# tsurumeso/vocal-remover

Measured on NVIDIA H100. Metric: seconds-of-audio/sec separated (n_fft=2048, hop=1024), higher is better.
Workload: dtype bf16x3 (split-bf16 operands hi+lo, 3 wgmma passes, fp32 accumulate); fft/lstm fp32

## Files before the change

vocal-remover_b200/build.py:

```python
import os
import subprocess
import sys
from concurrent.futures import ThreadPoolExecutor

HERE = os.path.dirname(os.path.abspath(__file__))
CSRC = os.path.join(HERE, 'csrc')
OBJ = os.path.join(HERE, 'build')
LIB = os.path.join(HERE, 'libvr_b200.so')
SOURCES = ['api.cu', 'engine.cu', 'conv_simt.cu', 'conv_tc.cu', 'conv_tc_rows.cu', 'elementwise.cu', 'lstm.cu', 'fft.cu', 'resample.cu']
NVCC = os.environ.get('NVCC', '/usr/local/cuda/bin/nvcc')
FLAGS = ['-gencode', 'arch=compute_90a,code=sm_90a', '-O3', '-lineinfo', '-std=c++17',
         '-Xcompiler', '-fPIC', '-Xcompiler', '-fvisibility=hidden', '--expt-relaxed-constexpr']


def _newest_header():
    hs = [os.path.join(CSRC, f) for f in os.listdir(CSRC) if f.endswith(('.h', '.cuh'))]
    hs.append(os.path.join(HERE, '..', 'include', 'vr_b200.h'))
    return max(os.path.getmtime(h) for h in hs)


def build(verbose=False, force=False):
    global OBJ, LIB
    extra = os.environ.get('VR_BUILD_FLAGS', '').split()
    if os.environ.get('VR_BUILD_TAG'):
        OBJ = os.path.join(HERE, 'build_' + os.environ['VR_BUILD_TAG'])
        LIB = os.path.join(HERE, 'libvr_b200_%s.so' % os.environ['VR_BUILD_TAG'])
    os.makedirs(OBJ, exist_ok=True)
    hdr = _newest_header()
    jobs = []
    for src in SOURCES:
        s = os.path.join(CSRC, src)
        o = os.path.join(OBJ, src.replace('.cu', '.o'))
        if force or not os.path.exists(o) or os.path.getmtime(o) < max(os.path.getmtime(s), hdr):
            jobs.append((s, o))

    def cc(job):
        s, o = job
        cmd = [NVCC] + FLAGS + extra + ['-c', s, '-o', o]
        if verbose:
            cmd += ['-Xptxas', '-v']
        r = subprocess.run(cmd, capture_output=True, text=True)
        if r.returncode != 0:
            raise RuntimeError('nvcc failed for %s:\n%s\n%s' % (s, r.stdout, r.stderr))
        return r.stderr

    with ThreadPoolExecutor(max_workers=min(8, max(1, len(jobs)))) as ex:
        logs = list(ex.map(cc, jobs))
    if verbose:
        for lg in logs:
            print(lg)
    objs = [os.path.join(OBJ, s.replace('.cu', '.o')) for s in SOURCES]
    if jobs or not os.path.exists(LIB):
        cmd = [NVCC, '-shared', '-o', LIB] + objs + ['-gencode', 'arch=compute_90a,code=sm_90a']
        r = subprocess.run(cmd, capture_output=True, text=True)
        if r.returncode != 0:
            raise RuntimeError('link failed:\n%s\n%s' % (r.stdout, r.stderr))
    return LIB


if __name__ == '__main__':
    print(build(verbose='-v' in sys.argv, force='-f' in sys.argv))
```

vocal-remover_b200/csrc/conv_tc.cu:

```cuda
#include <cuda.h>
#include <stdio.h>

#include <map>
#include <tuple>

#include "engine.h"
#include "tc_common.cuh"
#include "tc_plan.h"

namespace vr {

static constexpr int kMaxStages = 8;
static constexpr int kConsumerWarps = 8;
static constexpr int kThreads = 32 * kConsumerWarps + 32;

struct TcParams {
  int N, Ho, Wo, Wt, Ht, Nt, tiles_w, tiles_h, m_tiles, n_tiles;
  int stride, pad_h, pad_w, dil_h, dil_w, KW;
  int cchunks, total_sub, CinPadTC, Cout, act, stages;
  bf16* out_hi;
  bf16* out_lo;
  int64_t osn, osh;
  int osw;
  const float* bias;
// ... 117 lines not shown
        if (++stage == p.stages) {
          stage = 0;
          phase ^= 1u;
        }
      }
      wg_wait<0>();
      __syncwarp();
      if (lane == 0) mbar_arrive(empty0 + (uint32_t)prev * 8u);

      const int nt = tile % p.n_tiles;
      const int mt = tile / p.n_tiles;
      const int w0 = (mt % p.tiles_w) * p.Wt;
      const int h0 = ((mt / p.tiles_w) % p.tiles_h) * p.Ht;
      const int n0 = (mt / (p.tiles_w * p.tiles_h)) * p.Nt;
      const int c_lane = nt * BN + 2 * (lane & 3);
#pragma unroll
      for (int hr = 0; hr < 2; ++hr) {
        const int row = 64 * wg + 16 * (warp & 3) + (lane >> 2) + 8 * hr;
        const int dw = row % p.Wt;
        const int dh = (row / p.Wt) % p.Ht;
        const int n = n0 + row / (p.Wt * p.Ht);
        if (n >= p.N) continue;
        const int64_t obase = (int64_t)n * p.osn + (int64_t)(h0 + dh) * p.osh + (int64_t)(w0 + dw) * p.osw;
#pragma unroll
        for (int j = 0; j < BN / 8; ++j)
          epilogue_pair(acc[4 * j + 2 * hr], acc[4 * j + 2 * hr + 1], bias_s, c_lane + 8 * j, p.Cout, slope,
                        p.out_hi + obase, p.out_lo + obase);
      }
    }
  }
}

#define VR_TC_FOR_BN(X, KB) X(KB, 16) X(KB, 32) X(KB, 48) X(KB, 64) X(KB, 80) X(KB, 96) X(KB, 112) X(KB, 128)
#define VR_TC_FOR_ALL(X) VR_TC_FOR_BN(X, 64) VR_TC_FOR_BN(X, 32) VR_TC_FOR_BN(X, 16)

int g_tc_debug[8] = {0, 0, 0, 0, 0, 1, 1, 0};

static constexpr int kMaxDevices = 64;
const TcDevice& tc_device() {
  static TcDevice table[kMaxDevices];
  static TcDevice none;
  int dev = -1;
  if (cudaGetDevice(&dev) != cudaSuccess || dev < 0 || dev >= kMaxDevices) return none;
  TcDevice& d = table[dev];
  if (!d.ok) {
    if (cudaDeviceGetAttribute(&d.max_smem, cudaDevAttrMaxSharedMemoryPerBlockOptin, dev) != cudaSuccess ||
        cudaDeviceGetAttribute(&d.num_sms, cudaDevAttrMultiProcessorCount, dev) != cudaSuccess)
      return none;
#define VR_TC_SET_SMEM(KB, BN) \
  cudaFuncSetAttribute(conv_tc_kernel<KB, BN>, cudaFuncAttributeMaxDynamicSharedMemorySize, d.max_smem - 2048);
    VR_TC_FOR_ALL(VR_TC_SET_SMEM)
#undef VR_TC_SET_SMEM
    tc_rows_set_attributes(d.max_smem);
    d.ok = true;
  }
  return d;
}

EncodeTiledFn tc_encode_fn() {
  static EncodeTiledFn fn = nullptr;
  if (!fn) {
    void* p = nullptr;
    cudaDriverEntryPointQueryResult q;
    if (cudaGetDriverEntryPoint("cuTensorMapEncodeTiled", &p, cudaEnableDefault, &q) == cudaSuccess &&
        q == cudaDriverEntryPointSuccess)
      fn = (EncodeTiledFn)p;
  }
  return fn;
}

static CUtensorMapSwizzle swizzle_for(int KB) {
  return KB == 64 ? CU_TENSOR_MAP_SWIZZLE_128B : KB == 32 ? CU_TENSOR_MAP_SWIZZLE_64B : CU_TENSOR_MAP_SWIZZLE_32B;
}

uint16_t tc_f2bf(float f) {
  uint32_t u;
  memcpy(&u, &f, 4);
  if ((u & 0x7fffffffu) > 0x7f800000u) return (uint16_t)((u >> 16) | 0x40);
  uint32_t r = 0x7fffu + ((u >> 16) & 1u);
  return (uint16_t)((u + r) >> 16);
}
float tc_bf2f(uint16_t h) {
  uint32_t u = (uint32_t)h << 16;
  float f;
  memcpy(&f, &u, 4);
  return f;
}

struct TileGeom {
  int Wt, Ht, Nt;
  bool ok;
};
static TileGeom tile_geom(int Ho, int Wo) {
  TileGeom g{0, 0, 0, false};
  if (Wo <= 0 || Ho <= 0) return g;
  if (Wo >= 128) {
    if (Wo % 128) return g;
    g.Wt = 128; g.Ht = 1; g.Nt = 1;
  } else {
    if (128 % Wo) return g;
    g.Wt = Wo;
    g.Ht = 128 / Wo < Ho ? 128 / Wo : Ho;
    if (Ho % g.Ht) return g;
    if ((128 / Wo) % g.Ht) return g;
    g.Nt = 128 / (g.Wt * g.Ht);
  }
// ... 27 lines not shown
  auto tc = std::make_shared<TcConv>();
  tc->taps = L.k * L.k;
  tc->CinPadTC = round_up(L.CinPad, 16);
  tc->KB = tc->CinPadTC % 64 == 0 ? 64 : tc->CinPadTC % 32 == 0 ? 32 : 16;
  tc->cchunks = tc->CinPadTC / tc->KB;
  tc->SUBS = 64 / tc->KB;
  tc->Ktot = tc->taps * tc->CinPadTC;
  tc->CoutPadN = round_up(L.Cout, 16);
  tc->n_tiles = ceil_div(tc->CoutPadN, 128);
  tc->BN = round_up(ceil_div(tc->CoutPadN, tc->n_tiles), 16);
  const int rows = tc->n_tiles * tc->BN;
  std::vector<uint16_t> planes((size_t)2 * rows * tc->Ktot, 0);
  for (int co = 0; co < L.Cout; ++co)
    for (int t = 0; t < tc->taps; ++t)
      for (int ci = 0; ci < L.CinPad; ++ci) {
        const float w = L.w_host[((size_t)t * L.CinPad + ci) * L.CoutPad + co];
        const uint16_t hi = tc_f2bf(w);
        const uint16_t lo = tc_f2bf(w - tc_bf2f(hi));
        const size_t k = (size_t)t * tc->CinPadTC + ci;
        planes[(size_t)co * tc->Ktot + k] = hi;
        planes[((size_t)rows + co) * tc->Ktot + k] = lo;
      }
  std::vector<float> bias((size_t)rows, 0.f);
  for (int co = 0; co < L.Cout; ++co) bias[(size_t)co] = L.bias_host[(size_t)co];
  void* dw = nullptr;
  void* db = nullptr;
  if (cudaMalloc(&dw, planes.size() * 2) != cudaSuccess || cudaMalloc(&db, bias.size() * 4) != cudaSuccess) {
    err = "cudaMalloc failed while packing tensor-core weights for " + L.name;
    return false;
  }
  allocs.push_back(dw);
  allocs.push_back(db);
  cudaMemcpy(dw, planes.data(), planes.size() * 2, cudaMemcpyHostToDevice);
  cudaMemcpy(db, bias.data(), bias.size() * 4, cudaMemcpyHostToDevice);
  tc->w_planes = (bf16*)dw;
  tc->bias = (float*)db;
  EncodeTiledFn enc = tc_encode_fn();
  if (!enc) {
    err = "cuTensorMapEncodeTiled is not available from the driver";
    return false;
  }
  cuuint64_t dims[3] = {(cuuint64_t)tc->Ktot, (cuuint64_t)rows, 2};
  cuuint64_t strides[2] = {(cuuint64_t)tc->Ktot * 2, (cuuint64_t)rows * tc->Ktot * 2};
  cuuint32_t box[3] = {(cuuint32_t)tc->KB, (cuuint32_t)tc->BN, 2};
  cuuint32_t es[3] = {1, 1, 1};
  CUresult r = enc(&tc->map_b, CU_TENSOR_MAP_DATA_TYPE_BFLOAT16, 3, dw, dims, strides, box, es,
                   CU_TENSOR_MAP_INTERLEAVE_NONE, swizzle_for(tc->KB), CU_TENSOR_MAP_L2_PROMOTION_L2_256B,
                   CU_TENSOR_MAP_FLOAT_OOB_FILL_NONE);
  if (r != CUDA_SUCCESS) {
    err = "cuTensorMapEncodeTiled(weights) failed for " + L.name + " code " + std::to_string((int)r);
    return false;
  }
  if (!tc_rows_prepare(L, *tc, err, allocs)) return false;
  L.tc = tc;
  return true;
}

cudaError_t tc_launch(ConvLayer& L, const ActView& in, const ActView& out, cudaStream_t s, std::string& err,
                      const ActView* up_src, const ActView* extra) {
  TcConv& tc = *L.tc;
  if (tc_rows_supported(L, tc, in, out)) return tc_rows_launch(L, tc, in, out, s, err, up_src, extra);
  if (up_src || extra) {
    err = "tc_launch: fused upsample is only implemented in the row-streaming kernel";
    return cudaErrorInvalidValue;
  }
  const TileGeom g = tile_geom(out.H, out.W);
  auto key = std::make_tuple((const void*)in.hi, (const void*)in.lo, in.N, in.H, in.W, in.C);
  auto it = tc.map_a.find(key);
  if (it == tc.map_a.end()) {
    CUtensorMap m;
    cuuint64_t dims[5] = {(cuuint64_t)in.C, (cuuint64_t)in.W, (cuuint64_t)in.H, (cuuint64_t)in.N, 2};
    const int64_t plane = (const char*)in.lo - (const char*)in.hi;
    if (plane <= 0 || plane % 16) {
      err = "tc_launch: hi/lo planes must be 16-byte aligned with lo after hi";
      return cudaErrorInvalidValue;
    }
    cuuint64_t strides[4] = {(cuuint64_t)in.sw * 2, (cuuint64_t)in.sh * 2, (cuuint64_t)in.sn * 2, (cuuint64_t)plane};
    cuuint32_t box[5] = {(cuuint32_t)tc.KB, (cuuint32_t)(g.Wt * L.stride), (cuuint32_t)(g.Ht * L.stride),
                         (cuuint32_t)g.Nt, 2};
    cuuint32_t es[5] = {1, (cuuint32_t)L.stride, (cuuint32_t)L.stride, 1, 1};
    CUresult r = tc_encode_fn()(&m, CU_TENSOR_MAP_DATA_TYPE_BFLOAT16, 5, (void*)in.hi, dims, strides, box, es,
                             CU_TENSOR_MAP_INTERLEAVE_NONE, swizzle_for(tc.KB), CU_TENSOR_MAP_L2_PROMOTION_L2_256B,
                             CU_TENSOR_MAP_FLOAT_OOB_FILL_NONE);
    if (r != CUDA_SUCCESS) {
      err = "cuTensorMapEncodeTiled(activations) failed for " + L.name + " code " + std::to_string((int)r);
      return cudaErrorInvalidValue;
    }
    it = tc.map_a.emplace(key, m).first;
  }
  TcParams p;
  p.N = out.N; p.Ho = out.H; p.Wo = out.W;
  p.Wt = g.Wt; p.Ht = g.Ht; p.Nt = g.Nt;
  p.tiles_w = out.W / g.Wt; p.tiles_h = out.H / g.Ht;
  p.m_tiles = p.tiles_w * p.tiles_h * ceil_div(out.N, g.Nt);
  p.n_tiles = tc.n_tiles;
  p.stride = L.stride; p.dil_h = L.dil_h; p.dil_w = L.dil_w;
  p.pad_h = L.dil_h * (L.k / 2); p.pad_w = L.dil_w * (L.k / 2);
  p.KW = L.k;
  p.cchunks = tc.cchunks; p.total_sub = tc.taps * tc.cchunks;
  p.CinPadTC = tc.CinPadTC; p.Cout = L.Cout; p.act = L.act;
  const int stage_bytes = tc.SUBS * (2 * 128 * tc.KB * 2 + 2 * tc.BN * tc.KB * 2);
  const TcDevice& dv = tc_device();
  if (!dv.ok) {
    err = "tc_launch: cannot query the current device";
    return cudaErrorInvalidValue;
  }
  const int dyn = dv.max_smem - 2048;
  p.stages = (dyn - 1024) / stage_bytes;
  if (p.stages > kMaxStages) p.stages = kMaxStages;
  if (p.stages < 2) {
    err = "tc_launch: shared memory too small for two pipeline stages";
    return cudaErrorInvalidValue;
  }
  p.out_hi = out.hi; p.out_lo = out.lo;
  p.osn = out.sn; p.osh = out.sh; p.osw = out.sw;
  p.bias = tc.bias;
  const int total_tiles = p.m_tiles * p.n_tiles;
  const int grid = total_tiles < dv.num_sms ? total_tiles : dv.num_sms;
// ... 13 lines not shown
```

vocal-remover_b200/csrc/conv_tc_rows.cu:

```cuda
#include <stdio.h>

#include "engine.h"
#include "tc_common.cuh"
#include "tc_plan.h"

namespace vr {

static constexpr int kInterpWarps = 10;
static constexpr int kConsumerWarps = 8;
static constexpr int kTmaWarp = kConsumerWarps;
static constexpr int kInterpWarp0 = kConsumerWarps + 1;
static constexpr int kMaxR = 8;
__host__ __device__ constexpr int rows_per_tile(int BN) { return BN == 64 ? 2 : BN == 32 ? 4 : 8; }
static constexpr int kUpProducerWarps = 12;
static constexpr int kUpConsumerRegs = 128;
static constexpr int kUpProducerRegs = 72;
static constexpr int kUpLaunchRegs = 96;
static_assert(kConsumerWarps * kUpConsumerRegs + kUpProducerWarps * kUpProducerRegs <=
                  (kConsumerWarps + kUpProducerWarps) * kUpLaunchRegs,
              "setmaxnreg.inc would wait forever for registers the block does not own");
__host__ __device__ constexpr int rows_threads(bool up) { return 32 * (kConsumerWarps + (up ? kUpProducerWarps : 1)); }
static constexpr int kRowPx = 130;
static constexpr int kBoxPx = 136;
static constexpr int kMaxASlots = 8;
static constexpr int kSrcPx = 68;
static constexpr uint32_t kKB = 32;
static constexpr uint32_t kRowB = kKB * 2;
static constexpr uint32_t kAPlane = kBoxPx * kRowB;
static constexpr uint32_t kASlot = 2 * kAPlane;

static constexpr int kTraceEvents = 2048;
__device__ unsigned long long g_rows_trace[3 * kTraceEvents * 3];

template <int BN>
struct RowsGeom {
  static constexpr uint32_t kBPlane = 3 * BN * kRowB;
  static constexpr uint32_t kBKw = 2 * kBPlane;
  static constexpr uint32_t kBBuf = 3 * kBKw;
};

struct RowsParams {
  int N, H, W, tiles_w, tiles_h, n_tiles, total_tiles;
  int chunks, CinPadR, Cout, act;
  int n_aslots;
  bf16* out_hi;
  bf16* out_lo;
  int64_t osn, osh;
  int osw;
  const float* bias;
  int up_chunks, xH, xW;
  const bf16* x_hi;
  const bf16* x_lo;
  int64_t xsn, xsh;
  int xsw;
  int trace;
  unsigned long long kmask;
  int a_c_off;
  int l_chunk;
  int n_uslots;
  float up_sh, up_sw;
  const float* dot_w;
  float* dot_out;
};

__device__ __forceinline__ uint32_t chunk_groups(unsigned long long kmask, int cc) {
  const int sh = cc * 4;
  return sh + 4 <= 64 ? (uint32_t)(kmask >> sh) & 0xFu : 0xFu;
}

struct RowsConsumer {
  int as_t, as_u, bs, as, pend_b;
  uint32_t aph_t, aph_u, bph, aph;
  int ring_lo, ring_hi;
};

template <int BN, int R, int r>
__device__ __forceinline__ void consume_rows(RowsConsumer& st, float* acc, uint32_t (&fr)[2][16], uint32_t lrow,
                                             uint32_t bsrc, uint32_t dhi, uint32_t ksm, uint32_t afull0,
                                             uint32_t aempty0, uint32_t bempty0, int lane) {
  constexpr int o_lo = r - 2 < 0 ? 0 : r - 2;
  constexpr int o_hi = r > R - 1 ? R - 1 : r;
  mbar_wait(afull0 + (uint32_t)st.as * 8u, st.aph);
  const uint32_t row = lrow + (uint32_t)st.as * kASlot;
#pragma unroll
  for (int kw = 0; kw < 3; ++kw) {
    uint32_t* f = fr[(3 * r + kw) & 1];
    const uint32_t q = (row >> 6) + (uint32_t)kw;
#pragma unroll
    for (int ks = 0; ks < 2; ++ks) {
      if (!((ksm >> ks) & 1u)) continue;
      const uint32_t a = (q << 6) + ((((uint32_t)(2 * ks) + ((uint32_t)lane >> 4)) ^ ((q >> 1) & 3u)) << 4);
      ldsm_x4(f + 8 * ks, a);
      ldsm_x4(f + 8 * ks + 4, a + kAPlane);
    }
    wg_fence();
#pragma unroll
    for (int ks = 0; ks < 2; ++ks) {
      if (!((ksm >> ks) & 1u)) continue;
      const uint32_t bo = (uint32_t)(kw * RowsGeom<BN>::kBKw + ks * 32) >> 4;
#pragma unroll
      for (int o = o_lo; o <= o_hi; ++o) {
        const uint32_t b_row = bsrc + (((uint32_t)((2 - (r - o)) * BN) * kRowB) >> 4) + bo;
        wgmma_split3_rs<BN>(acc + o * (BN / 2), f + 8 * ks, f + 8 * ks + 4, b_row,
                            b_row + (RowsGeom<BN>::kBPlane >> 4), dhi);
      }
    }
    wg_commit();
    if (kw == 2) {
      __syncwarp();
      if (lane == 0) mbar_arrive(aempty0 + (uint32_t)st.as * 8u);
    }
    wg_wait<1>();
    if (st.pend_b >= 0) {
      __syncwarp();
      if (lane == 0) mbar_arrive(bempty0 + (uint32_t)st.pend_b * 8u);
      st.pend_b = -1;
    }
  }
  if (++st.as == st.ring_hi) {
    st.as = st.ring_lo;
    st.aph ^= 1u;
// ... 543 lines not shown
```

vocal-remover_b200/csrc/tc_common.cuh:

```cuda
#pragma once
#include <cuda.h>
#include <stdint.h>
#include <stdio.h>

#include "common.cuh"

namespace vr {

__device__ __forceinline__ uint32_t smem_u32(const void* p) { return (uint32_t)__cvta_generic_to_shared(p); }

__device__ __forceinline__ bool elect_one_sync() {
  uint32_t pred;
  asm volatile(
      "{\n\t"
      ".reg .pred P1;\n\t"
      "elect.sync _|P1, 0xffffffff;\n\t"
      "selp.u32 %0, 1, 0, P1;\n\t"
      "}"
      : "=r"(pred));
  return pred != 0;
}

__device__ __forceinline__ void mbar_init(uint32_t bar, uint32_t count) {
  asm volatile("mbarrier.init.shared::cta.b64 [%0], %1;" ::"r"(bar), "r"(count));
// ... 130 lines not shown
  }
};
template <>
struct Wgmma<112> {
  static __device__ __forceinline__ void mma(float* d, uint64_t a, uint64_t b) {
    asm volatile(
        "wgmma.mma_async.sync.aligned.m64n112k16.f32.bf16.bf16 {%0, %1, %2, %3, %4, %5, %6, %7, %8, %9, %10, %11, %12, %13, %14, %15, %16, %17, %18, %19, %20, %21, %22, %23, %24, %25, %26, %27, %28, %29, %30, %31, %32, %33, %34, %35, %36, %37, %38, %39, %40, %41, %42, %43, %44, %45, %46, %47, %48, %49, %50, %51, %52, %53, %54, %55}, %56, %57, 1, 1, 1, 0, 0;"
        : "+f"(d[0]), "+f"(d[1]), "+f"(d[2]), "+f"(d[3]), "+f"(d[4]), "+f"(d[5]), "+f"(d[6]), "+f"(d[7]), "+f"(d[8]), "+f"(d[9]), "+f"(d[10]), "+f"(d[11]), "+f"(d[12]), "+f"(d[13]), "+f"(d[14]), "+f"(d[15]), "+f"(d[16]), "+f"(d[17]), "+f"(d[18]), "+f"(d[19]), "+f"(d[20]), "+f"(d[21]), "+f"(d[22]), "+f"(d[23]), "+f"(d[24]), "+f"(d[25]), "+f"(d[26]), "+f"(d[27]), "+f"(d[28]), "+f"(d[29]), "+f"(d[30]), "+f"(d[31]), "+f"(d[32]), "+f"(d[33]), "+f"(d[34]), "+f"(d[35]), "+f"(d[36]), "+f"(d[37]), "+f"(d[38]), "+f"(d[39]), "+f"(d[40]), "+f"(d[41]), "+f"(d[42]), "+f"(d[43]), "+f"(d[44]), "+f"(d[45]), "+f"(d[46]), "+f"(d[47]), "+f"(d[48]), "+f"(d[49]), "+f"(d[50]), "+f"(d[51]), "+f"(d[52]), "+f"(d[53]), "+f"(d[54]), "+f"(d[55])
        : "l"(a), "l"(b)
        : "memory");
  }
};
template <>
struct Wgmma<128> {
  static __device__ __forceinline__ void mma(float* d, uint64_t a, uint64_t b) {
    asm volatile(
        "wgmma.mma_async.sync.aligned.m64n128k16.f32.bf16.bf16 {%0, %1, %2, %3, %4, %5, %6, %7, %8, %9, %10, %11, %12, %13, %14, %15, %16, %17, %18, %19, %20, %21, %22, %23, %24, %25, %26, %27, %28, %29, %30, %31, %32, %33, %34, %35, %36, %37, %38, %39, %40, %41, %42, %43, %44, %45, %46, %47, %48, %49, %50, %51, %52, %53, %54, %55, %56, %57, %58, %59, %60, %61, %62, %63}, %64, %65, 1, 1, 1, 0, 0;"
        : "+f"(d[0]), "+f"(d[1]), "+f"(d[2]), "+f"(d[3]), "+f"(d[4]), "+f"(d[5]), "+f"(d[6]), "+f"(d[7]), "+f"(d[8]), "+f"(d[9]), "+f"(d[10]), "+f"(d[11]), "+f"(d[12]), "+f"(d[13]), "+f"(d[14]), "+f"(d[15]), "+f"(d[16]), "+f"(d[17]), "+f"(d[18]), "+f"(d[19]), "+f"(d[20]), "+f"(d[21]), "+f"(d[22]), "+f"(d[23]), "+f"(d[24]), "+f"(d[25]), "+f"(d[26]), "+f"(d[27]), "+f"(d[28]), "+f"(d[29]), "+f"(d[30]), "+f"(d[31]), "+f"(d[32]), "+f"(d[33]), "+f"(d[34]), "+f"(d[35]), "+f"(d[36]), "+f"(d[37]), "+f"(d[38]), "+f"(d[39]), "+f"(d[40]), "+f"(d[41]), "+f"(d[42]), "+f"(d[43]), "+f"(d[44]), "+f"(d[45]), "+f"(d[46]), "+f"(d[47]), "+f"(d[48]), "+f"(d[49]), "+f"(d[50]), "+f"(d[51]), "+f"(d[52]), "+f"(d[53]), "+f"(d[54]), "+f"(d[55]), "+f"(d[56]), "+f"(d[57]), "+f"(d[58]), "+f"(d[59]), "+f"(d[60]), "+f"(d[61]), "+f"(d[62]), "+f"(d[63])
        : "l"(a), "l"(b)
        : "memory");
  }
};
template <int N>
__device__ __forceinline__ void wgmma_split3(float* d, uint32_t a_hi, uint32_t a_lo, uint32_t b_hi, uint32_t b_lo,
                                             uint32_t dhi) {
  Wgmma<N>::mma(d, desc64(a_hi, dhi), desc64(b_hi, dhi));
  Wgmma<N>::mma(d, desc64(a_lo, dhi), desc64(b_hi, dhi));
  Wgmma<N>::mma(d, desc64(a_hi, dhi), desc64(b_lo, dhi));
}

template <int N>
struct WgmmaRS;
template <>
struct WgmmaRS<16> {
  static __device__ __forceinline__ void mma(float* d, const uint32_t* a, uint64_t b) {
    asm volatile(
        "wgmma.mma_async.sync.aligned.m64n16k16.f32.bf16.bf16 {%0, %1, %2, %3, %4, %5, %6, %7}, {%8, %9, %10, %11}, %12, 1, 1, 1, 0;"
        : "+f"(d[0]), "+f"(d[1]), "+f"(d[2]), "+f"(d[3]), "+f"(d[4]), "+f"(d[5]), "+f"(d[6]), "+f"(d[7])
        : "r"(a[0]), "r"(a[1]), "r"(a[2]), "r"(a[3]), "l"(b)
        : "memory");
  }
};
template <>
struct WgmmaRS<32> {
  static __device__ __forceinline__ void mma(float* d, const uint32_t* a, uint64_t b) {
    asm volatile(
        "wgmma.mma_async.sync.aligned.m64n32k16.f32.bf16.bf16 {%0, %1, %2, %3, %4, %5, %6, %7, %8, %9, %10, %11, %12, %13, %14, %15}, {%16, %17, %18, %19}, %20, 1, 1, 1, 0;"
        : "+f"(d[0]), "+f"(d[1]), "+f"(d[2]), "+f"(d[3]), "+f"(d[4]), "+f"(d[5]), "+f"(d[6]), "+f"(d[7]), "+f"(d[8]), "+f"(d[9]), "+f"(d[10]), "+f"(d[11]), "+f"(d[12]), "+f"(d[13]), "+f"(d[14]), "+f"(d[15])
        : "r"(a[0]), "r"(a[1]), "r"(a[2]), "r"(a[3]), "l"(b)
        : "memory");
  }
};
template <>
struct WgmmaRS<64> {
  static __device__ __forceinline__ void mma(float* d, const uint32_t* a, uint64_t b) {
    asm volatile(
        "wgmma.mma_async.sync.aligned.m64n64k16.f32.bf16.bf16 {%0, %1, %2, %3, %4, %5, %6, %7, %8, %9, %10, %11, %12, %13, %14, %15, %16, %17, %18, %19, %20, %21, %22, %23, %24, %25, %26, %27, %28, %29, %30, %31}, {%32, %33, %34, %35}, %36, 1, 1, 1, 0;"
        : "+f"(d[0]), "+f"(d[1]), "+f"(d[2]), "+f"(d[3]), "+f"(d[4]), "+f"(d[5]), "+f"(d[6]), "+f"(d[7]), "+f"(d[8]), "+f"(d[9]), "+f"(d[10]), "+f"(d[11]), "+f"(d[12]), "+f"(d[13]), "+f"(d[14]), "+f"(d[15]), "+f"(d[16]), "+f"(d[17]), "+f"(d[18]), "+f"(d[19]), "+f"(d[20]), "+f"(d[21]), "+f"(d[22]), "+f"(d[23]), "+f"(d[24]), "+f"(d[25]), "+f"(d[26]), "+f"(d[27]), "+f"(d[28]), "+f"(d[29]), "+f"(d[30]), "+f"(d[31])
        : "r"(a[0]), "r"(a[1]), "r"(a[2]), "r"(a[3]), "l"(b)
        : "memory");
  }
};
template <int N>
__device__ __forceinline__ void wgmma_split3_rs(float* d, const uint32_t* a_hi, const uint32_t* a_lo, uint32_t b_hi,
                                                uint32_t b_lo, uint32_t dhi) {
  WgmmaRS<N>::mma(d, a_hi, desc64(b_hi, dhi));
  WgmmaRS<N>::mma(d, a_lo, desc64(b_hi, dhi));
  WgmmaRS<N>::mma(d, a_hi, desc64(b_lo, dhi));
}

__device__ __forceinline__ void ldsm_x4(uint32_t* r, uint32_t addr) {
  asm volatile("ldmatrix.sync.aligned.m8n8.x4.shared.b16 {%0, %1, %2, %3}, [%4];"
               : "=r"(r[0]), "=r"(r[1]), "=r"(r[2]), "=r"(r[3])
               : "r"(addr)
               : "memory");
}

template <int N>
__device__ __forceinline__ void setmaxnreg_inc() {
  asm volatile("setmaxnreg.inc.sync.aligned.u32 %0;" ::"n"(N));
}
template <int N>
__device__ __forceinline__ void setmaxnreg_dec() {
  asm volatile("setmaxnreg.dec.sync.aligned.u32 %0;" ::"n"(N));
}

__device__ __forceinline__ void epilogue_pair(float v0, float v1, const float* bias_s, int c, int Cout, float slope,
                                              bf16* out_hi, bf16* out_lo) {
  if (c >= Cout) return;
  const float t0 = v0 + bias_s[c], t1 = v1 + bias_s[c + 1];
  const float y0 = fmaxf(t0, 0.f) + slope * fminf(t0, 0.f);
  const float y1 = fmaxf(t1, 0.f) + slope * fminf(t1, 0.f);
  bf16* h = out_hi + c;
  bf16* l = out_lo + c;
  if (c + 1 < Cout && ((reinterpret_cast<uintptr_t>(h) | reinterpret_cast<uintptr_t>(l)) & 3) == 0) {
    const uint32_t uh = f2_to_bf2(y0, y1);
    const float2 hf = bf2_to_f2(uh);
    *reinterpret_cast<uint32_t*>(h) = uh;
    *reinterpret_cast<uint32_t*>(l) = f2_to_bf2(y0 - hf.x, y1 - hf.y);
  } else {
    split_bf16(y0, h[0], l[0]);
    if (c + 1 < Cout) split_bf16(y1, h[1], l[1]);
  }
}

__device__ __forceinline__ void tma_load_4d(uint32_t dst, const CUtensorMap* map, int c0, int c1, int c2, int c3,
                                            uint32_t bar) {
  asm volatile(
      "cp.async.bulk.tensor.4d.shared::cluster.global.tile.mbarrier::complete_tx::bytes [%0], [%1, {%2, %3, %4, %5}], "
      "[%6];" ::"r"(dst),
      "l"(map), "r"(c0), "r"(c1), "r"(c2), "r"(c3), "r"(bar)
      : "memory");
}

}
```

vocal-remover_b200/csrc/tc_plan.h:

```cpp
#pragma once
#include <cuda.h>

#include <map>
#include <tuple>

#include "engine.h"

namespace vr {

typedef std::tuple<const void*, const void*, int, int, int, int> ViewKey;

struct TcRowsPlan {
  bool ok = false;
  int KB = 32, CinPadR = 0, chunks = 0, BN = 0, n_tiles = 0;
  unsigned long long kmask = ~0ull;
  bf16* w_planes = nullptr;
  float* bias = nullptr;
  CUtensorMap map_b;
  std::map<ViewKey, CUtensorMap> map_a;
  std::map<ViewKey, CUtensorMap> map_l;
};

struct TcConv {
  int CinPadTC = 0, KB = 0, cchunks = 0, SUBS = 0, taps = 0, Ktot = 0, CoutPadN = 0, BN = 0, n_tiles = 0;
  bf16* w_planes = nullptr;
  float* bias = nullptr;
  CUtensorMap map_b;
  std::map<ViewKey, CUtensorMap> map_a;
  TcRowsPlan rows;
};

typedef CUresult (*EncodeTiledFn)(CUtensorMap*, CUtensorMapDataType, cuuint32_t, void*, const cuuint64_t*,
                                  const cuuint64_t*, const cuuint32_t*, const cuuint32_t*, CUtensorMapInterleave,
                                  CUtensorMapSwizzle, CUtensorMapL2promotion, CUtensorMapFloatOOBfill);
EncodeTiledFn tc_encode_fn();
uint16_t tc_f2bf(float f);
float tc_bf2f(uint16_t h);

bool tc_rows_prepare(ConvLayer& L, TcConv& tc, std::string& err, std::vector<void*>& allocs);
bool tc_rows_supported(const ConvLayer& L, const TcConv& tc, const ActView& in, const ActView& out);
cudaError_t tc_rows_launch(ConvLayer& L, TcConv& tc, const ActView& in, const ActView& out, cudaStream_t s,
                           std::string& err, const ActView* up_src = nullptr, const ActView* extra = nullptr);
void tc_rows_set_attributes(int max_smem);
int tc_rows_read_trace(unsigned long long* out, long long capacity);

struct TcDevice {
  bool ok = false;
  int num_sms = 0, max_smem = 0;
};
const TcDevice& tc_device();

extern int g_tc_debug[8];

}
```

Before: 2613.

## Add halo-tile 3x3 conv kernel reusing one activation tile across all nine taps

Adds a new warp-specialized tensor-core kernel for 3x3 stride-1 convs on narrow widths (16/32/64). It loads one halo tile per channel chunk via TMA, builds all nine tap fragments from shared memory with ldmatrix, and streams the weights through a deep stage ring. This replaces per-tap re-fetching of activations in the generic implicit-GEMM path. It also chooses between one and two M-blocks per tile based on wave count. The new path is untested on other shapes, carries a large register budget, and adds more template instantiations.

```diff
diff --git a/vocal-remover_b200/build.py b/vocal-remover_b200/build.py
--- a/vocal-remover_b200/build.py
+++ b/vocal-remover_b200/build.py
@@ -7,7 +7,7 @@
 CSRC = os.path.join(HERE, 'csrc')
 OBJ = os.path.join(HERE, 'build')
 LIB = os.path.join(HERE, 'libvr_b200.so')
-SOURCES = ['api.cu', 'engine.cu', 'conv_simt.cu', 'conv_tc.cu', 'conv_tc_rows.cu', 'elementwise.cu', 'lstm.cu', 'fft.cu', 'resample.cu']
+SOURCES = ['api.cu', 'engine.cu', 'conv_simt.cu', 'conv_tc.cu', 'conv_tc_rows.cu', 'conv_tc_halo.cu', 'elementwise.cu', 'lstm.cu', 'fft.cu', 'resample.cu']
 NVCC = os.environ.get('NVCC', '/usr/local/cuda/bin/nvcc')
 FLAGS = ['-gencode', 'arch=compute_90a,code=sm_90a', '-O3', '-lineinfo', '-std=c++17',
          '-Xcompiler', '-fPIC', '-Xcompiler', '-fvisibility=hidden', '--expt-relaxed-constexpr']
diff --git a/vocal-remover_b200/csrc/conv_tc.cu b/vocal-remover_b200/csrc/conv_tc.cu
--- a/vocal-remover_b200/csrc/conv_tc.cu
+++ b/vocal-remover_b200/csrc/conv_tc.cu
@@ -193,6 +193,7 @@
     VR_TC_FOR_ALL(VR_TC_SET_SMEM)
 #undef VR_TC_SET_SMEM
     tc_rows_set_attributes(d.max_smem);
+    tc_halo_set_attributes(d.max_smem);
     d.ok = true;
   }
   return d;
@@ -326,6 +327,7 @@
     return false;
   }
   if (!tc_rows_prepare(L, *tc, err, allocs)) return false;
+  if (!tc_halo_prepare(L, *tc, err, allocs)) return false;
   L.tc = tc;
   return true;
 }
@@ -338,6 +340,7 @@
     err = "tc_launch: fused upsample is only implemented in the row-streaming kernel";
     return cudaErrorInvalidValue;
   }
+  if (tc_halo_supported(L, tc, in, out)) return tc_halo_launch(L, tc, in, out, s, err);
   const TileGeom g = tile_geom(out.H, out.W);
   auto key = std::make_tuple((const void*)in.hi, (const void*)in.lo, in.N, in.H, in.W, in.C);
   auto it = tc.map_a.find(key);
diff --git a/vocal-remover_b200/csrc/conv_tc_halo.cu b/vocal-remover_b200/csrc/conv_tc_halo.cu
--- /dev/null
+++ b/vocal-remover_b200/csrc/conv_tc_halo.cu
@@ -0,0 +1,372 @@
+#include <stdio.h>
+
+#include "engine.h"
+#include "tc_common.cuh"
+#include "tc_plan.h"
+
+namespace vr {
+
+static constexpr int kConsumerWarps = 8;
+static constexpr int kProducerWarps = 4;
+static constexpr int kThreads = 32 * (kConsumerWarps + kProducerWarps);
+static constexpr int kLaunchRegs = 168;
+static constexpr int kConsumerRegs = 232;
+static constexpr int kProducerRegs = 40;
+static_assert(kConsumerWarps * kConsumerRegs + kProducerWarps * kProducerRegs <=
+                  (kConsumerWarps + kProducerWarps) * kLaunchRegs,
+              "setmaxnreg.inc would wait forever for registers the block does not own");
+static constexpr int kMaxHSlots = 4;
+static constexpr int kMaxWStages = 18;
+static constexpr uint32_t kKB = 32;
+static constexpr uint32_t kRowB = kKB * 2;
+
+template <int BN>
+struct HaloGeom {
+  static constexpr uint32_t kBPlane = BN * kRowB;
+  static constexpr uint32_t kWStage = 2 * kBPlane;
+};
+
+struct HaloParams {
+  int N, H, W, lw, Ht, Wb, tiles_h, n_tiles, total_tiles;
+  int chunks, CinPadH, Cout, act;
+  int n_hslots, n_wstages;
+  uint32_t hplane, hslot;
+  unsigned long long kmask;
+  bf16* out_hi;
+  bf16* out_lo;
+  int64_t osn, osh;
+  int osw;
+  const float* bias;
+};
+
+struct HaloConsumer {
+  int hs, ws, pend_w;
+  uint32_t hph, wph;
+};
+
+template <int BN, int MB>
+__device__ __forceinline__ void consume_halo(HaloConsumer& st, const HaloParams& p, float* acc,
+                                             uint32_t (&fr)[2][MB * 8], const uint32_t* q0, uint32_t h_base,
+                                             uint32_t w_base, uint32_t dhi, uint32_t hfull0,
+                                             uint32_t hempty0, uint32_t wfull0, uint32_t wempty0, int lane) {
+  typedef HaloGeom<BN> G;
+  mbar_wait(hfull0 + (uint32_t)st.hs * 8u, st.hph);
+  const uint32_t slot = h_base + (uint32_t)st.hs * p.hslot;
+#pragma unroll
+  for (int t = 0; t < 9; ++t) {
+    const int kh = t / 3, kw = t % 3;
+#pragma unroll
+    for (int ks = 0; ks < 2; ++ks) {
+      uint32_t* f = fr[ks];
+#pragma unroll
+      for (int b = 0; b < MB; ++b) {
+        const uint32_t q = q0[b] + (uint32_t)(kh * p.Wb + kw);
+        const uint32_t a = slot + (q << 6) + ((((uint32_t)(2 * ks) + ((uint32_t)lane >> 4)) ^ ((q >> 1) & 3u)) << 4);
+        ldsm_x4(f + 8 * b, a);
+        ldsm_x4(f + 8 * b + 4, a + p.hplane);
+      }
+      if (ks == 0) mbar_wait(wfull0 + (uint32_t)st.ws * 8u, st.wph);
+      const uint32_t b_hi = desc_lo(w_base + (uint32_t)st.ws * G::kWStage) + (uint32_t)(ks * 32 >> 4);
+      wg_fence();
+#pragma unroll
+      for (int b = 0; b < MB; ++b)
+        wgmma_split3_rs<BN>(acc + b * (BN / 2), f + 8 * b, f + 8 * b + 4, b_hi, b_hi + (G::kBPlane >> 4), dhi);
+      wg_commit();
+      if (t == 8 && ks == 1) {
+        __syncwarp();
+        if (lane == 0) mbar_arrive(hempty0 + (uint32_t)st.hs * 8u);
+      }
+      wg_wait<1>();
+      if (st.pend_w >= 0) {
+        __syncwarp();
+        if (lane == 0) mbar_arrive(wempty0 + (uint32_t)st.pend_w * 8u);
+        st.pend_w = -1;
+      }
+    }
+    st.pend_w = st.ws;
+    if (++st.ws == p.n_wstages) {
+      st.ws = 0;
+      st.wph ^= 1u;
+    }
+  }
+  if (++st.hs == p.n_hslots) {
+    st.hs = 0;
+    st.hph ^= 1u;
+  }
+}
+
+template <int BN, int MB>
+__global__ void __launch_bounds__(kThreads, 1)
+    conv_tc_halo_kernel(const __grid_constant__ CUtensorMap tmA, const __grid_constant__ CUtensorMap tmB,
+                        const HaloParams p) {
+  typedef HaloGeom<BN> G;
+  extern __shared__ uint8_t smem_raw[];
+  __shared__ __align__(8) uint64_t bar_hfull[kMaxHSlots];
+  __shared__ __align__(8) uint64_t bar_hempty[kMaxHSlots];
+  __shared__ __align__(8) uint64_t bar_wfull[kMaxWStages];
+  __shared__ __align__(8) uint64_t bar_wempty[kMaxWStages];
+  __shared__ float bias_s[256];
+
+  const int warp = __shfl_sync(0xffffffffu, (int)threadIdx.x >> 5, 0);
+  const int lane = threadIdx.x & 31;
+  const uint32_t smem_base = (smem_u32(smem_raw) + 1023u) & ~1023u;
+  const uint32_t h_base = smem_base;
+  const uint32_t w_base = smem_base + (uint32_t)p.n_hslots * p.hslot;
+
+  if (warp == kConsumerWarps && lane == 0) {
+    asm volatile("prefetch.tensormap [%0];" ::"l"(&tmA) : "memory");
+    asm volatile("prefetch.tensormap [%0];" ::"l"(&tmB) : "memory");
+    for (int s = 0; s < p.n_hslots; ++s) {
+      mbar_init(smem_u32(&bar_hfull[s]), 1);
+      mbar_init(smem_u32(&bar_hempty[s]), kConsumerWarps);
+    }
+    for (int s = 0; s < p.n_wstages; ++s) {
+      mbar_init(smem_u32(&bar_wfull[s]), 1);
+      mbar_init(smem_u32(&bar_wempty[s]), kConsumerWarps);
+    }
+    asm volatile("fence.mbarrier_init.release.cluster;" ::: "memory");
+  }
+  for (int i = threadIdx.x; i < p.n_tiles * BN; i += blockDim.x) bias_s[i] = __ldg(p.bias + i);
+  __syncthreads();
+  const uint32_t hfull0 = smem_u32(&bar_hfull[0]), hempty0 = smem_u32(&bar_hempty[0]);
+  const uint32_t wfull0 = smem_u32(&bar_wfull[0]), wempty0 = smem_u32(&bar_wempty[0]);
+
+  if (warp >= kConsumerWarps) {
+    setmaxnreg_dec<kProducerRegs>();
+    if (warp == kConsumerWarps && elect_one_sync()) {
+      int hs = 0, ws = 0;
+      uint32_t hph = 0, wph = 0;
+      for (int tile = blockIdx.x; tile < p.total_tiles; tile += gridDim.x) {
+        const int nt = tile % p.n_tiles;
+        const int mt = tile / p.n_tiles;
+        const int h0 = (mt % p.tiles_h) * p.Ht;
+        const int n = mt / p.tiles_h;
+        for (int cc = 0; cc < p.chunks; ++cc) {
+          if (!chunk_groups(p.kmask, cc)) continue;
+          mbar_wait(hempty0 + (uint32_t)hs * 8u, hph ^ 1u);
+          const uint32_t hfull = hfull0 + (uint32_t)hs * 8u;
+          mbar_expect_tx(hfull, p.hslot);
+          tma_load_5d(h_base + (uint32_t)hs * p.hslot, &tmA, cc * (int)kKB, -1, h0 - 1, n, 0, hfull);
+          if (++hs == p.n_hslots) {
+            hs = 0;
+            hph ^= 1u;
+          }
+          for (int t = 0; t < 9; ++t) {
+            mbar_wait(wempty0 + (uint32_t)ws * 8u, wph ^ 1u);
+            const uint32_t wfull = wfull0 + (uint32_t)ws * 8u;
+            mbar_expect_tx(wfull, G::kWStage);
+            tma_load_3d(w_base + (uint32_t)ws * G::kWStage, &tmB, t * p.CinPadH + cc * (int)kKB, nt * BN, 0, wfull);
+            if (++ws == p.n_wstages) {
+              ws = 0;
+              wph ^= 1u;
+            }
+          }
+        }
+      }
+    }
+    __syncwarp();
+  } else {
+    setmaxnreg_inc<kConsumerRegs>();
+    const int wg = warp >> 2;
+    const float slope = p.act == ACT_RELU ? 0.f : p.act == ACT_LEAKY ? 0.01f : 1.f;
+    const uint32_t dhi = desc_hi(8 * kRowB, 2u);
+    uint32_t q0[MB];
+#pragma unroll
+    for (int b = 0; b < MB; ++b) {
+      const int px = 64 * (MB * wg + b) + 16 * (warp & 3) + (lane & 15);
+      q0[b] = (uint32_t)((px >> p.lw) * p.Wb + (px & (p.W - 1)));
+    }
+    HaloConsumer st;
+    st.hs = 0; st.ws = 0; st.pend_w = -1;
+    st.hph = 0; st.wph = 0;
+    float acc[MB * BN / 2];
+    uint32_t fr[2][MB * 8];
+    for (int tile = blockIdx.x; tile < p.total_tiles; tile += gridDim.x) {
+#pragma unroll
+      for (int i = 0; i < MB * BN / 2; ++i) acc[i] = 0.f;
+      for (int cc = 0; cc < p.chunks; ++cc) {
+        if (!chunk_groups(p.kmask, cc)) continue;
+        consume_halo<BN, MB>(st, p, acc, fr, q0, h_base, w_base, dhi, hfull0, hempty0, wfull0, wempty0, lane);
+      }
+      wg_wait<0>();
+      __syncwarp();
+      if (lane == 0 && st.pend_w >= 0) mbar_arrive(wempty0 + (uint32_t)st.pend_w * 8u);
+      st.pend_w = -1;
+
+      const int nt = tile % p.n_tiles;
+      const int mt = tile / p.n_tiles;
+      const int h0 = (mt % p.tiles_h) * p.Ht;
+      const int n = mt / p.tiles_h;
+      const int c_lane = nt * BN + 2 * (lane & 3);
+#pragma unroll
+      for (int b = 0; b < MB; ++b) {
+#pragma unroll
+        for (int hr = 0; hr < 2; ++hr) {
+          const int px = 64 * (MB * wg + b) + 16 * (warp & 3) + (lane >> 2) + 8 * hr;
+          const int64_t obase =
+              (int64_t)n * p.osn + (int64_t)(h0 + (px >> p.lw)) * p.osh + (int64_t)(px & (p.W - 1)) * p.osw;
+          const float* v = acc + b * (BN / 2) + 2 * hr;
+#pragma unroll
+          for (int j = 0; j < BN / 8; ++j)
+            epilogue_pair(v[4 * j], v[4 * j + 1], bias_s, c_lane + 8 * j, p.Cout, slope, p.out_hi + obase,
+                          p.out_lo + obase);
+        }
+      }
+    }
+  }
+}
+
+#define VR_HALO_FOR_MB(X, BN) X(BN, 1) X(BN, 2)
+#define VR_HALO_FOR_ALL(X) \
+  VR_HALO_FOR_MB(X, 16) VR_HALO_FOR_MB(X, 32) VR_HALO_FOR_MB(X, 48) VR_HALO_FOR_MB(X, 64) VR_HALO_FOR_MB(X, 96) \
+  VR_HALO_FOR_MB(X, 128)
+
+static bool halo_has_bn(int BN) { return BN == 16 || BN == 32 || BN == 48 || BN == 64 || BN == 96 || BN == 128; }
+
+bool tc_halo_prepare(ConvLayer& L, TcConv& tc, std::string& err, std::vector<void*>& allocs) {
+  TcHaloPlan& Hp = tc.halo;
+  Hp.ok = false;
+  if (L.k != 3 || L.stride != 1 || L.dil_h != 1 || L.dil_w != 1 || !halo_has_bn(tc.BN)) return true;
+  if (tc.n_tiles * tc.BN > 256) return true;
+  Hp.CinPadH = round_up(L.CinPad, (int)kKB);
+  Hp.chunks = Hp.CinPadH / (int)kKB;
+  const int rows = tc.n_tiles * tc.BN;
+  const int Ktot = 9 * Hp.CinPadH;
+  std::vector<uint16_t> planes((size_t)2 * rows * Ktot, 0);
+  for (int co = 0; co < L.Cout; ++co)
+    for (int t = 0; t < 9; ++t)
+      for (int ci = 0; ci < L.CinPad; ++ci) {
+        const float w = L.w_host[((size_t)t * L.CinPad + ci) * L.CoutPad + co];
+        const uint16_t hi = tc_f2bf(w);
+        const uint16_t lo = tc_f2bf(w - tc_bf2f(hi));
+        const size_t k = (size_t)t * Hp.CinPadH + ci;
+        planes[(size_t)co * Ktot + k] = hi;
+        planes[((size_t)rows + co) * Ktot + k] = lo;
+      }
+  Hp.kmask = ~0ull;
+  if (Hp.CinPadH / 8 <= 64) {
+    Hp.kmask = 0x3ull;
+    for (int ci = 0; ci < L.CinPad; ++ci) {
+      bool any = false;
+      for (int t = 0; t < 9 && !any; ++t)
+        for (int co = 0; co < L.Cout && !any; ++co) any = L.w_host[((size_t)t * L.CinPad + ci) * L.CoutPad + co] != 0.f;
+      if (any) Hp.kmask |= 1ull << (ci / 8);
+    }
+  }
+  void* dw = nullptr;
+  if (cudaMalloc(&dw, planes.size() * 2) != cudaSuccess) {
+    err = "cudaMalloc failed while packing halo-kernel weights for " + L.name;
+    return false;
+  }
+  allocs.push_back(dw);
+  cudaMemcpy(dw, planes.data(), planes.size() * 2, cudaMemcpyHostToDevice);
+  Hp.w_planes = (bf16*)dw;
+  cuuint64_t dims[3] = {(cuuint64_t)Ktot, (cuuint64_t)rows, 2};
+  cuuint64_t strides[2] = {(cuuint64_t)Ktot * 2, (cuuint64_t)rows * Ktot * 2};
+  cuuint32_t box[3] = {kKB, (cuuint32_t)tc.BN, 2};
+  cuuint32_t es[3] = {1, 1, 1};
+  CUresult r = tc_encode_fn()(&Hp.map_b, CU_TENSOR_MAP_DATA_TYPE_BFLOAT16, 3, dw, dims, strides, box, es,
+                              CU_TENSOR_MAP_INTERLEAVE_NONE, CU_TENSOR_MAP_SWIZZLE_64B,
+                              CU_TENSOR_MAP_L2_PROMOTION_L2_256B, CU_TENSOR_MAP_FLOAT_OOB_FILL_NONE);
+  if (r != CUDA_SUCCESS) {
+    err = "cuTensorMapEncodeTiled(halo-kernel weights) failed for " + L.name + " code " + std::to_string((int)r);
+    return false;
+  }
+  Hp.ok = true;
+  return true;
+}
+
+bool tc_halo_supported(const ConvLayer& L, const TcConv& tc, const ActView& in, const ActView& out) {
+  if (!tc.halo.ok || g_tc_debug[3] == 1) return false;
+  if (L.k != 3 || L.stride != 1 || L.dil_h != 1 || L.dil_w != 1) return false;
+  if (!(out.W == 16 || out.W == 32 || out.W == 64) || in.H != out.H || in.W != out.W) return false;
+  if (out.H % (128 / out.W)) return false;
+  if (in.sw % 8 || in.sh % 8 || in.sn % 8) return false;
+  if ((reinterpret_cast<uintptr_t>(in.hi) | reinterpret_cast<uintptr_t>(in.lo)) & 15) return false;
+  return in.C > 0 && in.N > 0;
+}
+
+cudaError_t tc_halo_launch(ConvLayer& L, TcConv& tc, const ActView& in, const ActView& out, cudaStream_t s,
+                           std::string& err) {
+  TcHaloPlan& Hp = tc.halo;
+  const TcDevice& dv = tc_device();
+  if (!dv.ok) {
+    err = "tc_halo_launch: cannot query the current device";
+    return cudaErrorInvalidValue;
+  }
+  const int ht1 = 128 / out.W;
+  const bool mb2_tiles = out.H % (2 * ht1) == 0;
+  const int tiles1 = out.N * (out.H / ht1) * tc.n_tiles;
+  const int waves1 = ceil_div(tiles1, dv.num_sms), waves2 = ceil_div(tiles1 / 2, dv.num_sms);
+  int MB = mb2_tiles && 19 * waves2 <= 10 * waves1 ? 2 : 1;
+  if (g_tc_debug[3] == 2) MB = 1;
+  if (g_tc_debug[3] == 3 && mb2_tiles) MB = 2;
+  HaloParams p;
+  p.N = out.N; p.H = out.H; p.W = out.W;
+  p.lw = out.W == 16 ? 4 : out.W == 32 ? 5 : 6;
+  p.Ht = MB * ht1;
+  p.Wb = round_up(out.W + 2, 8);
+  p.tiles_h = out.H / p.Ht;
+  p.n_tiles = tc.n_tiles;
+  p.total_tiles = out.N * p.tiles_h * p.n_tiles;
+  p.chunks = Hp.chunks; p.CinPadH = Hp.CinPadH; p.Cout = L.Cout; p.act = L.act;
+  p.hplane = (uint32_t)((p.Ht + 2) * p.Wb) * kRowB;
+  p.hslot = 2 * p.hplane;
+  p.kmask = g_tc_debug[6] == 1 ? Hp.kmask : ~0ull;
+  p.out_hi = out.hi; p.out_lo = out.lo;
+  p.osn = out.sn; p.osh = out.sh; p.osw = out.sw;
+  p.bias = tc.bias;
+  ViewKey key = std::make_tuple((const void*)in.hi, (const void*)in.lo, in.N, in.H, in.W, in.C);
+  auto it = Hp.map_a[MB - 1].find(key);
+  if (it == Hp.map_a[MB - 1].end()) {
+    CUtensorMap m;
+    const int64_t plane = (const char*)in.lo - (const char*)in.hi;
+    if (plane <= 0 || plane % 16) {
+      err = "tc_halo_launch: hi/lo planes must be 16-byte aligned with lo after hi";
+      return cudaErrorInvalidValue;
+    }
+    cuuint64_t dims[5] = {(cuuint64_t)in.C, (cuuint64_t)in.W, (cuuint64_t)in.H, (cuuint64_t)in.N, 2};
+    cuuint64_t strides[4] = {(cuuint64_t)in.sw * 2, (cuuint64_t)in.sh * 2, (cuuint64_t)in.sn * 2, (cuuint64_t)plane};
+    cuuint32_t box[5] = {kKB, (cuuint32_t)p.Wb, (cuuint32_t)(p.Ht + 2), 1, 2};
+    cuuint32_t es[5] = {1, 1, 1, 1, 1};
+    CUresult r = tc_encode_fn()(&m, CU_TENSOR_MAP_DATA_TYPE_BFLOAT16, 5, (void*)in.hi, dims, strides, box, es,
+                                CU_TENSOR_MAP_INTERLEAVE_NONE, CU_TENSOR_MAP_SWIZZLE_64B,
+                                CU_TENSOR_MAP_L2_PROMOTION_L2_256B, CU_TENSOR_MAP_FLOAT_OOB_FILL_NONE);
+    if (r != CUDA_SUCCESS) {
+      err = "cuTensorMapEncodeTiled(halo-kernel activations) failed for " + L.name + " code " + std::to_string((int)r);
+      return cudaErrorInvalidValue;
+    }
+    it = Hp.map_a[MB - 1].emplace(key, m).first;
+  }
+  const int w_stage = tc.BN * 2 * (int)kRowB;
+  const int dyn = dv.max_smem - 2048;
+  const int avail = dyn - 1024;
+  p.n_hslots = (avail - 9 * w_stage) / (int)p.hslot;
+  if (p.n_hslots > kMaxHSlots) p.n_hslots = kMaxHSlots;
+  if (p.n_hslots < 2) p.n_hslots = 2;
+  p.n_wstages = (avail - p.n_hslots * (int)p.hslot) / w_stage;
+  if (p.n_wstages > kMaxWStages) p.n_wstages = kMaxWStages;
+  if (p.n_wstages < 2) {
+    err = "tc_halo_launch: shared memory too small for two halo slots and two weight stages";
+    return cudaErrorInvalidValue;
+  }
+  const int grid = p.total_tiles < dv.num_sms ? p.total_tiles : dv.num_sms;
+#define VR_HALO_LAUNCH(BN_, MB_)                                                           \
+  if (tc.BN == BN_ && MB == MB_) {                                                         \
+    conv_tc_halo_kernel<BN_, MB_><<<grid, kThreads, dyn, s>>>(it->second, Hp.map_b, p);   \
+    return cudaGetLastError();                                                             \
+  }
+  VR_HALO_FOR_ALL(VR_HALO_LAUNCH)
+#undef VR_HALO_LAUNCH
+  err = "tc_halo_launch: no kernel instantiation for this channel tile";
+  return cudaErrorInvalidValue;
+}
+
+void tc_halo_set_attributes(int max_smem) {
+#define VR_HALO_SET(BN_, MB_) \
+  cudaFuncSetAttribute(conv_tc_halo_kernel<BN_, MB_>, cudaFuncAttributeMaxDynamicSharedMemorySize, max_smem - 2048);
+  VR_HALO_FOR_ALL(VR_HALO_SET)
+#undef VR_HALO_SET
+}
+
+}
diff --git a/vocal-remover_b200/csrc/conv_tc_rows.cu b/vocal-remover_b200/csrc/conv_tc_rows.cu
--- a/vocal-remover_b200/csrc/conv_tc_rows.cu
+++ b/vocal-remover_b200/csrc/conv_tc_rows.cu
@@ -62,11 +62,6 @@
   const float* dot_w;
   float* dot_out;
 };
-
-__device__ __forceinline__ uint32_t chunk_groups(unsigned long long kmask, int cc) {
-  const int sh = cc * 4;
-  return sh + 4 <= 64 ? (uint32_t)(kmask >> sh) & 0xFu : 0xFu;
-}
 
 struct RowsConsumer {
   int as_t, as_u, bs, as, pend_b;
diff --git a/vocal-remover_b200/csrc/tc_common.cuh b/vocal-remover_b200/csrc/tc_common.cuh
--- a/vocal-remover_b200/csrc/tc_common.cuh
+++ b/vocal-remover_b200/csrc/tc_common.cuh
@@ -206,11 +206,41 @@
   }
 };
 template <>
+struct WgmmaRS<48> {
+  static __device__ __forceinline__ void mma(float* d, const uint32_t* a, uint64_t b) {
+    asm volatile(
+        "wgmma.mma_async.sync.aligned.m64n48k16.f32.bf16.bf16 {%0, %1, %2, %3, %4, %5, %6, %7, %8, %9, %10, %11, %12, %13, %14, %15, %16, %17, %18, %19, %20, %21, %22, %23}, {%24, %25, %26, %27}, %28, 1, 1, 1, 0;"
+        : "+f"(d[0]), "+f"(d[1]), "+f"(d[2]), "+f"(d[3]), "+f"(d[4]), "+f"(d[5]), "+f"(d[6]), "+f"(d[7]), "+f"(d[8]), "+f"(d[9]), "+f"(d[10]), "+f"(d[11]), "+f"(d[12]), "+f"(d[13]), "+f"(d[14]), "+f"(d[15]), "+f"(d[16]), "+f"(d[17]), "+f"(d[18]), "+f"(d[19]), "+f"(d[20]), "+f"(d[21]), "+f"(d[22]), "+f"(d[23])
+        : "r"(a[0]), "r"(a[1]), "r"(a[2]), "r"(a[3]), "l"(b)
+        : "memory");
+  }
+};
+template <>
 struct WgmmaRS<64> {
   static __device__ __forceinline__ void mma(float* d, const uint32_t* a, uint64_t b) {
     asm volatile(
         "wgmma.mma_async.sync.aligned.m64n64k16.f32.bf16.bf16 {%0, %1, %2, %3, %4, %5, %6, %7, %8, %9, %10, %11, %12, %13, %14, %15, %16, %17, %18, %19, %20, %21, %22, %23, %24, %25, %26, %27, %28, %29, %30, %31}, {%32, %33, %34, %35}, %36, 1, 1, 1, 0;"
         : "+f"(d[0]), "+f"(d[1]), "+f"(d[2]), "+f"(d[3]), "+f"(d[4]), "+f"(d[5]), "+f"(d[6]), "+f"(d[7]), "+f"(d[8]), "+f"(d[9]), "+f"(d[10]), "+f"(d[11]), "+f"(d[12]), "+f"(d[13]), "+f"(d[14]), "+f"(d[15]), "+f"(d[16]), "+f"(d[17]), "+f"(d[18]), "+f"(d[19]), "+f"(d[20]), "+f"(d[21]), "+f"(d[22]), "+f"(d[23]), "+f"(d[24]), "+f"(d[25]), "+f"(d[26]), "+f"(d[27]), "+f"(d[28]), "+f"(d[29]), "+f"(d[30]), "+f"(d[31])
+        : "r"(a[0]), "r"(a[1]), "r"(a[2]), "r"(a[3]), "l"(b)
+        : "memory");
+  }
+};
+template <>
+struct WgmmaRS<96> {
+  static __device__ __forceinline__ void mma(float* d, const uint32_t* a, uint64_t b) {
+    asm volatile(
+        "wgmma.mma_async.sync.aligned.m64n96k16.f32.bf16.bf16 {%0, %1, %2, %3, %4, %5, %6, %7, %8, %9, %10, %11, %12, %13, %14, %15, %16, %17, %18, %19, %20, %21, %22, %23, %24, %25, %26, %27, %28, %29, %30, %31, %32, %33, %34, %35, %36, %37, %38, %39, %40, %41, %42, %43, %44, %45, %46, %47}, {%48, %49, %50, %51}, %52, 1, 1, 1, 0;"
+        : "+f"(d[0]), "+f"(d[1]), "+f"(d[2]), "+f"(d[3]), "+f"(d[4]), "+f"(d[5]), "+f"(d[6]), "+f"(d[7]), "+f"(d[8]), "+f"(d[9]), "+f"(d[10]), "+f"(d[11]), "+f"(d[12]), "+f"(d[13]), "+f"(d[14]), "+f"(d[15]), "+f"(d[16]), "+f"(d[17]), "+f"(d[18]), "+f"(d[19]), "+f"(d[20]), "+f"(d[21]), "+f"(d[22]), "+f"(d[23]), "+f"(d[24]), "+f"(d[25]), "+f"(d[26]), "+f"(d[27]), "+f"(d[28]), "+f"(d[29]), "+f"(d[30]), "+f"(d[31]), "+f"(d[32]), "+f"(d[33]), "+f"(d[34]), "+f"(d[35]), "+f"(d[36]), "+f"(d[37]), "+f"(d[38]), "+f"(d[39]), "+f"(d[40]), "+f"(d[41]), "+f"(d[42]), "+f"(d[43]), "+f"(d[44]), "+f"(d[45]), "+f"(d[46]), "+f"(d[47])
+        : "r"(a[0]), "r"(a[1]), "r"(a[2]), "r"(a[3]), "l"(b)
+        : "memory");
+  }
+};
+template <>
+struct WgmmaRS<128> {
+  static __device__ __forceinline__ void mma(float* d, const uint32_t* a, uint64_t b) {
+    asm volatile(
+        "wgmma.mma_async.sync.aligned.m64n128k16.f32.bf16.bf16 {%0, %1, %2, %3, %4, %5, %6, %7, %8, %9, %10, %11, %12, %13, %14, %15, %16, %17, %18, %19, %20, %21, %22, %23, %24, %25, %26, %27, %28, %29, %30, %31, %32, %33, %34, %35, %36, %37, %38, %39, %40, %41, %42, %43, %44, %45, %46, %47, %48, %49, %50, %51, %52, %53, %54, %55, %56, %57, %58, %59, %60, %61, %62, %63}, {%64, %65, %66, %67}, %68, 1, 1, 1, 0;"
+        : "+f"(d[0]), "+f"(d[1]), "+f"(d[2]), "+f"(d[3]), "+f"(d[4]), "+f"(d[5]), "+f"(d[6]), "+f"(d[7]), "+f"(d[8]), "+f"(d[9]), "+f"(d[10]), "+f"(d[11]), "+f"(d[12]), "+f"(d[13]), "+f"(d[14]), "+f"(d[15]), "+f"(d[16]), "+f"(d[17]), "+f"(d[18]), "+f"(d[19]), "+f"(d[20]), "+f"(d[21]), "+f"(d[22]), "+f"(d[23]), "+f"(d[24]), "+f"(d[25]), "+f"(d[26]), "+f"(d[27]), "+f"(d[28]), "+f"(d[29]), "+f"(d[30]), "+f"(d[31]), "+f"(d[32]), "+f"(d[33]), "+f"(d[34]), "+f"(d[35]), "+f"(d[36]), "+f"(d[37]), "+f"(d[38]), "+f"(d[39]), "+f"(d[40]), "+f"(d[41]), "+f"(d[42]), "+f"(d[43]), "+f"(d[44]), "+f"(d[45]), "+f"(d[46]), "+f"(d[47]), "+f"(d[48]), "+f"(d[49]), "+f"(d[50]), "+f"(d[51]), "+f"(d[52]), "+f"(d[53]), "+f"(d[54]), "+f"(d[55]), "+f"(d[56]), "+f"(d[57]), "+f"(d[58]), "+f"(d[59]), "+f"(d[60]), "+f"(d[61]), "+f"(d[62]), "+f"(d[63])
         : "r"(a[0]), "r"(a[1]), "r"(a[2]), "r"(a[3]), "l"(b)
         : "memory");
   }
@@ -258,6 +288,11 @@
   }
 }
 
+__device__ __forceinline__ uint32_t chunk_groups(unsigned long long kmask, int cc) {
+  const int sh = cc * 4;
+  return sh + 4 <= 64 ? (uint32_t)(kmask >> sh) & 0xFu : 0xFu;
+}
+
 __device__ __forceinline__ void tma_load_4d(uint32_t dst, const CUtensorMap* map, int c0, int c1, int c2, int c3,
                                             uint32_t bar) {
   asm volatile(
diff --git a/vocal-remover_b200/csrc/tc_plan.h b/vocal-remover_b200/csrc/tc_plan.h
--- a/vocal-remover_b200/csrc/tc_plan.h
+++ b/vocal-remover_b200/csrc/tc_plan.h
@@ -21,6 +21,15 @@
   std::map<ViewKey, CUtensorMap> map_l;
 };
 
+struct TcHaloPlan {
+  bool ok = false;
+  int CinPadH = 0, chunks = 0;
+  unsigned long long kmask = ~0ull;
+  bf16* w_planes = nullptr;
+  CUtensorMap map_b;
+  std::map<ViewKey, CUtensorMap> map_a[2];
+};
+
 struct TcConv {
   int CinPadTC = 0, KB = 0, cchunks = 0, SUBS = 0, taps = 0, Ktot = 0, CoutPadN = 0, BN = 0, n_tiles = 0;
   bf16* w_planes = nullptr;
@@ -28,6 +37,7 @@
   CUtensorMap map_b;
   std::map<ViewKey, CUtensorMap> map_a;
   TcRowsPlan rows;
+  TcHaloPlan halo;
 };
 
 typedef CUresult (*EncodeTiledFn)(CUtensorMap*, CUtensorMapDataType, cuuint32_t, void*, const cuuint64_t*,
@@ -44,6 +54,12 @@
 void tc_rows_set_attributes(int max_smem);
 int tc_rows_read_trace(unsigned long long* out, long long capacity);
 
+bool tc_halo_prepare(ConvLayer& L, TcConv& tc, std::string& err, std::vector<void*>& allocs);
+bool tc_halo_supported(const ConvLayer& L, const TcConv& tc, const ActView& in, const ActView& out);
+cudaError_t tc_halo_launch(ConvLayer& L, TcConv& tc, const ActView& in, const ActView& out, cudaStream_t s,
+                           std::string& err);
+void tc_halo_set_attributes(int max_smem);
+
 struct TcDevice {
   bool ok = false;
   int num_sms = 0, max_smem = 0;
```

New measurement: 2706, median of 6. 1.04x the previous value.
